# albertfgu/diffwave-sashimi

Hardware: AMD Instinct MI355X
Metric: audio samples/sec (generate.py-style reverse-diffusion sampling, T=200) (higher is better)
Workload: dtype f32-equivalent (3-term bf16 split, 6 products, fp32 accumulate); 1 GPU; wnet_h256_d36_T200; backbone=wavenet, batch_per_gpu=16, L=16000, T=200, parallelism=independent clips per GPU, no collective, sampler=hipGraph replay, on-device Philox noise

## Files before the change

### diffwave-sashimi_amd/csrc/wavenet.h

```cpp
#pragma once
#include "dws_common.h"

namespace dws {

constexpr int WN_LAYER_KC = 32;
constexpr int WN_BX3_KC = 16;

struct WnLayerArgs {
    const float* x_in;
    float* x_out;
    float* skip;
    const float* part_t;
    int part_t_bstride;
    const float* A1;
    const float* A2;
    const float* Abt;
    int abt_bstride;
    const int* step_idx;
    int abt_tstride, part_t_tstride;
    const float* Wd;
    const float* Wr;
    const float* Ws;
    const float* bias1;
    const float* bias2;
// ... 20 lines not shown
    int af_scaled;
};

int launch_fold_weight_norm(const float* v, const float* g, float* out, int O, int inner, hipStream_t s);
int launch_permute_dconv(const float* w, float* out, int C, int KC, hipStream_t s);
int launch_pack_a_frag(const float* w, float* out, int M, int K, hipStream_t s);
int launch_pack_a_frag_t(const float* w, float* out, int O, int K, hipStream_t s);
int launch_step_embed(const float* steps, const float* freq, float* emb, int B, int half, hipStream_t s);
int launch_iota_f32(float* out, int n, hipStream_t s);
int launch_linear_rows(const float* in, const float* W, const float* bias, float* out, int B, int K, int O,
                       int act, hipStream_t s, float* pre_out = nullptr);
int launch_init_conv_bwd_data(const float* g, const float* y, const float* W, float* daudio, int B, int Cin, int C, int L,
                              hipStream_t s);
int launch_init_conv(const float* audio, const float* W, const float* bias, float* x, int B, int Cin, int C, int L,
                     hipStream_t s);
int launch_wn_bias_tap(const float* Wd_all, const float* part_t, float* Abt, int NL, int B, int C, hipStream_t s);
bool wn_layer_mfma_supported(int C, int S);
int launch_wn_layer_mfma(int C, int S, const WnLayerArgs& a, hipStream_t s);
int launch_wn_layer_generic(int C, int S, const WnLayerArgs& a, hipStream_t s);
bool wn_final_mfma_supported(int S);
bool wn_layer_wino_supported(int C, int S);
int launch_wino_dconv(const float* w, float* out, int C, hipStream_t s);
int launch_wn_wino_bias(const float* Wd_all, const float* part_t, float* Abt, int NL, int B, int C, hipStream_t s);
int launch_wn_layer_wino(int C, int S, const WnLayerArgs& a, hipStream_t s);
bool wn_layer_bf16x3_supported(int C, int S);
int launch_wn_layer_bf16x3(int C, int S, const WnLayerArgs& a, hipStream_t s);
int launch_pack_a_bf16x3(const float* w, void* out, int M, int K, hipStream_t s);
int launch_wn_bias_tap_bf16(const float* Wd_all, const float* part_t, const float* bias1_all, void* Abt, int NL, int B, int C,
                            hipStream_t s);
enum { WN_SPLIT_BF16X6 = 0, WN_SPLIT_F16X3 = 1 };
inline int wn_split_terms(int split) { return split == WN_SPLIT_F16X3 ? 2 : 3; }
enum { WN_BX6_MFMA_32 = 0, WN_BX6_MFMA_G2_16 = 1, WN_BX6_MFMA_16 = 2 };
constexpr int WN_BX6_MFMA_DEFAULT = WN_BX6_MFMA_16;
bool wn_layer_bx6_supported(int C, int S);
bool wn_layer_bx6_mfma16_supported(int C, int S, int split);
int launch_wn_layer_bx6(int C, int S, const WnLayerArgs& a, int split, int mfma, hipStream_t s);
int launch_weight_scale(const float* w, size_t n, const float* bias, int nb, const float* bias_b, int nb_b, float* out, hipStream_t s);
int launch_pack_a1_bx6(const float* w, void* out, int C, int split, const float* scale, hipStream_t s);
int launch_pack_a_bx6(const float* w, void* out, int M, int K, int split, const float* scale, hipStream_t s);
int launch_gemm_bx6(const float* A, const float* B, float* C, int M, int N, int K, int split, float sa, float sb, hipStream_t s);
int launch_wn_final(int S, const WnFinalArgs& a, hipStream_t s);

}
```

### diffwave-sashimi_amd/csrc/wavenet_bx6.hip

```cpp
#include <cstdlib>
#include <type_traits>

#include "bf16_split.h"
#include "wavenet.h"
#include "wn_trace.h"

namespace dws {

#ifndef BX6_PF3
#define BX6_PF3 1
#endif
#ifndef BX6_PF2
#define BX6_PF2 2
#endif
#define BX6_PF(NT) ((NT) == 2 ? BX6_PF2 : BX6_PF3)
#ifndef BX6_T_SLOTS
#define BX6_T_SLOTS 0, 2, 3, 4, 6, 7, 9
#endif

typedef float bx6_f32x4 __attribute__((ext_vector_type(4)));

#ifdef BX6_ABL_NO_NT
#define BX6_NT 0
#else
// ... 106 lines not shown
        hipLaunchKernelGGL(pack_a_bx6_kernel<SplitBf16x3>, dim3(ceil_div(n, 256)), dim3(256), 0, s, w, (unsigned short*)out, M, K, scale);
    }
    return DWS_OK;
}

template <int C, int S, int NT>
struct Bx6Tile {
    static constexpr int WAVES = C / 32;
    static constexpr int NTH = WAVES * 64;
    static constexpr int NP = 32;
    static constexpr int KC = (C >= 256) ? 32 : 16;
    static constexpr int NCB = C / KC;
    static constexpr int NKB = C / 16;
    static constexpr int MS = S / C;
    static constexpr int RAW_FLOATS = KC * 4 * NP;
    static constexpr int BOP_BYTES = (KC / 8) * 4 * NT * NP * 16;
    static constexpr int STAGE_FLOATS = 2 * RAW_FLOATS + 2 * BOP_BYTES / 4;
    static constexpr int GATE_BYTES = (C / 8) * NT * 64 * 16;
    static constexpr int MAIN_FLOATS = STAGE_FLOATS > GATE_BYTES / 4 ? STAGE_FLOATS : GATE_BYTES / 4;
    static constexpr int TR_FLOATS = 32 * 64;
    static constexpr int LDS_FLOATS = MAIN_FLOATS + WAVES * TR_FLOATS;
    static constexpr int TITEMS = (KC / 4) * NP * 2;
    static constexpr bool HALVES = WAVES == 8 && NT == 3;
    static constexpr int SW = HALVES ? WAVES / 2 : WAVES;
    static constexpr int NPIECE = KC / (2 * SW);
    static_assert(C % 32 == 0 && S % C == 0 && C % KC == 0 && KC % 16 == 0 && KC % (2 * SW) == 0 && (SW & (SW - 1)) == 0 &&
                  (!HALVES || NCB % 2 == 0) && (TITEMS % NTH == 0) && LDS_FLOATS * 4 <= 163840, "channel counts");
};

enum { BX6_MF_32 = 0, BX6_MF_G2_16 = 1, BX6_MF_16 = 2 };
#ifndef BX6_T16_SLOTS
#define BX6_T16_SLOTS 1, 5, 7, 9, 13, 15, 19
#endif
struct Bx6Nothing {};
template <int MS>
struct Bx6G2State {
    bx_f32x4 bias[1 + MS][2];
    bx_f32x4 acc[1 + MS][2][2][2];
};
template <int NT>
__device__ __forceinline__ int bx6_voff_a1h(int lane) { return ((lane >> 5) * (4 * NT * 64) + ((lane >> 4) & 1) * 32 + (lane & 15)) * 16; }
template <typename V8, int NT>
__device__ __forceinline__ void bx6_load_a1h(V8 (&dst)[2][NT], __amdgpu_buffer_rsrc_t r, int voff, int soff) {
#pragma unroll
    for (int h = 0; h < 2; ++h)
#pragma unroll
        for (int t = 0; t < NT; ++t) dst[h][t] = __builtin_bit_cast(V8, __builtin_amdgcn_raw_buffer_load_b128(r, voff + h * 256, soff + t * 1024, 0));
}
template <typename V8, int NT>
struct Bx6G1State {
    bx_f32x4 av[2][2][4], ab[2][2];
    bx_f32x4 acc[2][4][2][2];
    V8 ar[2][2][NT];
};
template <typename P, int C, int S, bool EXTRA, int MF = BX6_MF_32>
__global__ __launch_bounds__(C * 2, (C >= 128 ? 2 : 1)) void wn_layer_bx6_kernel(WnLayerArgs a, int log2d) {
    using T = Bx6Tile<C, S, P::NT>;
    static_assert(MF == BX6_MF_32 || (P::NT == 3 && !P::SCALED && C == 256 && S == 256), "the 16x16x32 shape: bf16 split, C = S = 256");
    using v8 = typename P::v8;
    using v4 = typename P::v4;
    constexpr int NT = P::NT, NPR = P::NP, NA = 2 * P::NT;
    constexpr int KC = T::KC, MS = T::MS, WAVES = T::WAVES, NCB = T::NCB, NTH = T::NTH, NKB = T::NKB;
    __shared__ __attribute__((aligned(16))) float lds[T::LDS_FLOATS];
    float* const Xraw = lds;
    char* const Bop = reinterpret_cast<char*>(lds + 2 * T::RAW_FLOATS);
    char* const gt = reinterpret_cast<char*>(lds);

    const int tid = threadIdx.x;
    const int lane = tid & 63;
    const int wave = __builtin_amdgcn_readfirstlane(tid >> 6);
    const int l31 = lane & 31, lhi = lane >> 5;
    const int L = a.L, dil = 1 << log2d;
    float* const trw = lds + T::MAIN_FLOATS + wave * T::TR_FLOATS;

    const int nblk = (L + 2 * dil - 1) >> (log2d + 1);
    const int ntl = ((nblk << log2d) + 31) >> 5;
    const int tile = xcd_remap(blockIdx.x, gridDim.x);
    const int b = __builtin_amdgcn_readfirstlane(tile / ntl);
    const int tic = tile % ntl;
#ifdef WN_TILE_ORDER_LINEAR
    const int q0 = __builtin_amdgcn_readfirstlane(tic * 32);
#else
    const int q0 = __builtin_amdgcn_readfirstlane(log2d >= 6 ? ((tic % nblk) << log2d) + (tic / nblk) * 32 : tic * 32);
#endif
    const int q = q0 + l31;
    const int p = ((q >> log2d) << (log2d + 1)) + (q & (dil - 1));

    const float* __restrict__ xb = a.x_in + (size_t)b * C * L;
    unsigned long long* __restrict__ trc = a.trace ? a.trace + ((size_t)blockIdx.x * WAVES + wave) * 32 : nullptr;
    auto stamp = [&](int i) {
        if (trc) {
// ... 150 lines not shown
    auto transform = [&](int c1) {
        TState ts;
#pragma unroll
        for (int u = 0; u < T_UNITS; ++u) transform_unit(c1, u, ts);
    };
    auto keep_residual = [&](int c1) {
        const int ch0 = chunk_of(c1) * KC;
        if (al16 && ch0 / 32 == wave) {
            const float* xs = Xraw + (c1 & 1) * T::RAW_FLOATS;
            const int r0 = ch0 % 32;
#pragma unroll
            for (int i = 0; i < KC / 4; ++i) {
                const int rr = (lane >> 4) + 4 * i;
                const bx6_f32x4 v = *reinterpret_cast<const bx6_f32x4*>(xs + rr * 128 + 32 + 4 * (lane & 15));
                *reinterpret_cast<bx6_f32x4*>(trw + (r0 + rr) * 64 + 4 * (lane & 15)) = v;
            }
        }
    };

    bx_f32x16 acc[2][4];
    __amdgpu_buffer_rsrc_t rA1 = __builtin_amdgcn_make_buffer_rsrc((void*)a.A1, 0, 2 * C * 4 * C * 2 * NT, 0x00020000);
    const int lane16 = lane * 16;
    auto load_a1 = [&](v8 (&dst)[2][NT], int kb, int j) {
#pragma unroll
        for (int m = 0; m < 2; ++m)
#pragma unroll
            for (int t = 0; t < NT; ++t)
#ifdef BX6_ABL_A_HOT
                dst[m][t] = __builtin_bit_cast(v8, __builtin_amdgcn_raw_buffer_load_b128(rA1, lane16, ((mt1[m] * NKB * 4) * NT + t) * 1024 + 0 * (kb + j), 0));
#else
                dst[m][t] = __builtin_bit_cast(v8, __builtin_amdgcn_raw_buffer_load_b128(rA1, lane16, (((mt1[m] * NKB + kb) * 4 + j) * NT + t) * 1024, 0));
#endif
    };

    if constexpr (MF >= BX6_MF_16) {
        static_assert(T::HALVES && NCB > 1 && BX6_PF(NT) == 1 && KC == 32,
                      "a wave stages chunk 0 or chunk 1; one half-step of six fragments ahead: NAF and the chunk loop's vmcnt counts as in the 32x32x16 form");
        bx6_load_a1h<v8, NT>(gs1.ar[0], rA1, bx6_voff_a1h<NT>(lane), ((mt1[0] * NKB + 2 * chunk_of(0)) * 4 + 0) * NT * 1024);
        stage_dma(shalf);
    } else {
    if (stages(0)) stage_dma(0);
    if (NCB > 1 && stages(1)) stage_dma(1);
    }
    constexpr int PF = BX6_PF(NT);
    v8 a_ring[4][2][NT];
    if constexpr (MF < BX6_MF_16) {
#pragma unroll
    for (int s0 = 0; s0 < PF; ++s0) load_a1(a_ring[s0], chunk_of(0) * (KC / 16) + (s0 >> 2), s0 & 3);
    }
    constexpr int NAF = PF * NA;
    constexpr int P16 = NPIECE + NAF, P4 = 4 * NPIECE + NAF;
    static_assert(P4 < 64, "vmcnt is a 6-bit counter");
    if constexpr (MF >= BX6_MF_16) {
        float bi[2][4];
#pragma unroll
        for (int c = 0; c < 2; ++c) {
            const int qc = q0 + 16 * c + (lane & 15);
            const int pc = ((qc >> log2d) << (log2d + 1)) + (qc & (dil - 1));
            const float v0 = ((unsigned)(pc - dil) < (unsigned)L) ? 1.f : 0.f;
            const float v1 = ((unsigned)pc < (unsigned)L) ? 1.f : 0.f;
            const float v2 = ((unsigned)(pc + dil) < (unsigned)L) ? 1.f : 0.f;
            const float v3 = ((unsigned)(pc + 2 * dil) < (unsigned)L) ? 1.f : 0.f;
            bi[c][0] = v0 - v2; bi[c][1] = v1 + v2; bi[c][2] = v2 - v1; bi[c][3] = v1 - v3;
        }
#pragma unroll
        for (int j = 0; j < 4; ++j)
#pragma unroll
            for (int m = 0; m < 2; ++m)
#pragma unroll
                for (int h = 0; h < 2; ++h)
#pragma unroll
// ... 90 lines not shown
#pragma unroll
            for (int m = 0; m < 2; ++m) {
                acc[m][j] = P::mfma(a_ring[st & 3][m][P::ia(t)], bq[P::ib(t)], acc[m][j]);
                if (ride) {
                    const int i = 2 * t + m;
#pragma unroll
                    for (int u = 0; u < T_UNITS; ++u)
                        if (T_SLOTS[NPR == 3 ? 0 : 1][u] == i) transform_unit(cb + 1, u, ts);
                    __builtin_amdgcn_sched_barrier(0);
                }
            }
    };
    auto do_steps_from1 = [&](int cb) {
        if constexpr (SPC == 4) {
            do_step(cb, std::integral_constant<int, 1>{}, std::false_type{});
            do_step(cb, std::integral_constant<int, 2>{}, std::false_type{});
            do_step(cb, std::integral_constant<int, 3>{}, std::false_type{});
        } else {
            do_step(cb, std::integral_constant<int, 1>{}, std::false_type{});
            do_step(cb, std::integral_constant<int, 2>{}, std::false_type{});
            do_step(cb, std::integral_constant<int, 3>{}, std::false_type{});
            do_step(cb, std::integral_constant<int, 4>{}, std::false_type{});
            do_step(cb, std::integral_constant<int, 5>{}, std::false_type{});
            do_step(cb, std::integral_constant<int, 6>{}, std::false_type{});
            do_step(cb, std::integral_constant<int, 7>{}, std::false_type{});
        }
    };
    static_assert((SPC == 4 || SPC == 8) && PF >= 1 && PF <= 3, "steps per chunk, prefetch distance");
    if constexpr (MF >= BX6_MF_16) {
        const int r16 = lane & 15, oct = lane >> 4;
        const int voffa = bx6_voff_a1h<NT>(lane);
        constexpr int T16_SLOTS[T_UNITS] = {BX6_T16_SLOTS};
        v8 bq[2][NT], bq0[2][2];
        auto do_half = [&](int cb, auto HS, auto WITH_T) {
            constexpr int hs = decltype(HS)::value, j = hs >> 1, m = hs & 1;
            constexpr bool ride = decltype(WITH_T)::value;
            const char* tb = Bop + (cb & 1) * T::BOP_BYTES + oct * (4 * NT * 512) + r16 * 16;
            if (hs == 2 && cb + 1 < NCB) keep_residual(cb + 1);
            if (hs < 7) bx6_load_a1h<v8, NT>(gs1.ar[(hs + 1) & 1], rA1, voffa, ((mt1[(hs + 1) & 1] * NKB + 2 * chunk_of(cb)) * 4 + ((hs + 1) >> 1)) * NT * 1024);
            else if (cb + 1 < NCB) bx6_load_a1h<v8, NT>(gs1.ar[0], rA1, voffa, ((mt1[0] * NKB + 2 * chunk_of(cb + 1)) * 4 + 0) * NT * 1024);
            __builtin_amdgcn_sched_barrier(0);
            if (hs == 0) {
#pragma unroll
                for (int t = 0; t < NT; ++t)
#pragma unroll
                    for (int c = 0; c < 2; ++c) (t ? bq[c][t] : bq0[0][c]) = *reinterpret_cast<const v8*>(tb + (j * NT + t) * 512 + c * 256);
            }
            if (m == 1 && j < 3) {
#pragma unroll
                for (int c = 0; c < 2; ++c) bq0[(j + 1) & 1][c] = *reinterpret_cast<const v8*>(tb + ((j + 1) * NT) * 512 + c * 256);
            }
            TState ts;
#pragma unroll
            for (int t = 0; t < NPR; ++t) {
#pragma unroll
                for (int h = 0; h < 2; ++h)
#pragma unroll
                    for (int c = 0; c < 2; ++c) {
                        gs1.acc[m][j][h][c] = P::mfma16(gs1.ar[hs & 1][h][P::ia(t)], P::ib(t) ? bq[c][P::ib(t)] : bq0[j & 1][c], gs1.acc[m][j][h][c]);
                        if (ride) {
                            const int i = (2 * t + h) * 2 + c;
#pragma unroll
                            for (int u = 0; u < T_UNITS; ++u)
                                if (T16_SLOTS[u] == i) transform_unit(cb + 1, u, ts);
                            __builtin_amdgcn_sched_barrier(0);
                        }
                    }
                if (m == 1 && j < 3 && (t == 2 || t == 4)) {
                    const int term = (t == 2) ? 2 : 1;
#pragma unroll
                    for (int c = 0; c < 2; ++c) bq[c][term] = *reinterpret_cast<const v8*>(tb + ((j + 1) * NT + term) * 512 + c * 256);
                }
            }
        };
        for (int cb = 0; cb < NCB; ++cb) {
            if (cb + 2 < NCB && stages(cb + 2)) stage_dma(cb + 2);
            if (cb + 1 < NCB) do_half(cb, std::integral_constant<int, 0>{}, std::true_type{});
            else do_half(cb, std::integral_constant<int, 0>{}, std::false_type{});
            do_half(cb, std::integral_constant<int, 1>{}, std::false_type{});
            do_half(cb, std::integral_constant<int, 2>{}, std::false_type{});
            do_half(cb, std::integral_constant<int, 3>{}, std::false_type{});
            do_half(cb, std::integral_constant<int, 4>{}, std::false_type{});
            do_half(cb, std::integral_constant<int, 5>{}, std::false_type{});
            do_half(cb, std::integral_constant<int, 6>{}, std::false_type{});
            do_half(cb, std::integral_constant<int, 7>{}, std::false_type{});
            stamp(8 + 2 * cb);
            __builtin_amdgcn_s_waitcnt(0x0F70 | NAF);
            __syncthreads();
            stamp(9 + 2 * cb);
        }
    } else {
    for (int cb = 0; cb < NCB; ++cb) {
#ifndef BX6_ABL_NO_STAGE
        if (cb + 2 < NCB && stages(cb + 2)) stage_dma(cb + 2);
#endif
        if (cb + 1 < NCB) do_step(cb, std::integral_constant<int, 0>{}, std::true_type{});
        else do_step(cb, std::integral_constant<int, 0>{}, std::false_type{});
        do_steps_from1(cb);
        stamp(8 + 2 * cb);
#ifndef BX6_ABL_NO_DMA_WAIT
        __builtin_amdgcn_s_waitcnt(0x0F70 | NAF);
#endif
#ifndef BX6_ABL_NO_BARRIER
        __syncthreads();
#endif
        stamp(9 + 2 * cb);
    }
    }
    stamp(2);
    int lane_t = lane;
    if constexpr (MF >= BX6_MF_16) asm volatile("" : "+v"(lane_t));

    [[maybe_unused]] std::conditional_t<MF >= BX6_MF_G2_16, Bx6G2State<MS>, Bx6Nothing> gs2;
    if constexpr (MF >= BX6_MF_G2_16) {
#pragma unroll
        for (int m = 0; m < 1 + MS; ++m)
#pragma unroll
            for (int h = 0; h < 2; ++h) gs2.bias[m][h] = *reinterpret_cast<const bx_f32x4*>(a.bias2 + mt2[m] * 32 + 16 * h + 4 * (lane_t >> 4));
    }
    const int L4 = L * 4;
    const bool first = a.first_layer, last = a.last_layer;
    __amdgpu_buffer_rsrc_t rXo = __builtin_amdgcn_make_buffer_rsrc((void*)(a.x_out + (size_t)b * C * L), 0, C * L * 4, 0x00020000);
// ... 319 lines not shown
        }
#pragma unroll
        for (int n = 0; n < 2; ++n) {
            if (!last) {
                const int s0 = (wave * 32) * L4;
#pragma unroll
                for (int r = 0; r < 16; ++r) {
                    const int so = s0 + ((r & 3) + 8 * (r >> 2)) * L4;
                    const float x = __builtin_bit_cast(float, __builtin_amdgcn_raw_buffer_load_b32(rXall, voffn[n], so, 0));
                    const float v = (x + (P::SCALED ? acc2[0][n][r] * inv2 : acc2[0][n][r])) * rs;
                    __builtin_amdgcn_raw_buffer_store_b32(__builtin_bit_cast(unsigned, v), rXo, voffn[n], so, 0);
                }
            }
#pragma unroll
            for (int m = 0; m < MS; ++m) {
                const int s0 = ((wave * MS + m) * 32) * L4;
#pragma unroll
                for (int r = 0; r < 16; ++r) {
                    const int so = s0 + ((r & 3) + 8 * (r >> 2)) * L4;
                    const float old = first ? 0.f : __builtin_bit_cast(float, __builtin_amdgcn_raw_buffer_load_b32(rSk, voffn[n], so, 0));
                    const float v = old + (P::SCALED ? acc2[1 + m][n][r] * inv2 : acc2[1 + m][n][r]);
                    __builtin_amdgcn_raw_buffer_store_b32(__builtin_bit_cast(unsigned, v), rSk, voffn[n], so, 0);
                }
            }
        }
    }
    stamp(6);
    if (trc) {
        __builtin_amdgcn_s_waitcnt(0);
        stamp(7);
    }
}

template <typename P, int C, int S, int MF = BX6_MF_32>
static int launch_bx6_t(const WnLayerArgs& a, int log2d, hipStream_t s) {
    ProfileScope ps(P::NT == 3 ? "wn_layer_bx6" : "wn_layer_f16x3", s);
    using T = Bx6Tile<C, S, P::NT>;
    const int dil = 1 << log2d;
    const int nblk = (a.L + 2 * dil - 1) / (2 * dil);
    const int ntl = (nblk * dil + 31) / 32;
    const int ntiles = a.B * ntl;
    static const bool trace = std::getenv("DWS_BX6_TRACE") != nullptr;
    if (trace && !a.melc && !a.hsave) {
        wino_trace_launch(ntiles, T::WAVES, a, s, [&](const WnLayerArgs& at) {
            hipLaunchKernelGGL((wn_layer_bx6_kernel<P, C, S, false, MF>), dim3(ntiles), dim3(T::NTH), 0, s, at, log2d);
        }, P::NT == 3 ? "bx6" : "f16x3");
        return DWS_OK;
    }
    if (a.melc || a.hsave) hipLaunchKernelGGL((wn_layer_bx6_kernel<P, C, S, true, MF>), dim3(ntiles), dim3(T::NTH), 0, s, a, log2d);
    else hipLaunchKernelGGL((wn_layer_bx6_kernel<P, C, S, false, MF>), dim3(ntiles), dim3(T::NTH), 0, s, a, log2d);
    return DWS_OK;
}

bool wn_layer_bx6_mfma16_supported(int C, int S, int split) { return split == WN_SPLIT_BF16X6 && C == 256 && S == 256; }

bool wn_layer_bx6_supported(int C, int S) {
    return (C == 64 && S == 64) || (C == 128 && S == 128) || (C == 128 && S == 256) || (C == 256 && S == 256);
}

template <typename P>
static int launch_bx6_p(int C, int S, const WnLayerArgs& a, int log2d, hipStream_t s) {
    if (C == 64 && S == 64) return launch_bx6_t<P, 64, 64>(a, log2d, s);
    if (C == 128 && S == 128) return launch_bx6_t<P, 128, 128>(a, log2d, s);
    if (C == 128 && S == 256) return launch_bx6_t<P, 128, 256>(a, log2d, s);
    if (C == 256 && S == 256) return launch_bx6_t<P, 256, 256>(a, log2d, s);
    return set_error(DWS_ERR_UNSUPPORTED, "wn_layer_bx6: (C=%d,S=%d) not instantiated", C, S);
}

int launch_wn_layer_bx6(int C, int S, const WnLayerArgs& a, int split, int mfma, hipStream_t s) {
    int log2d = 0;
    while ((1 << log2d) < a.dilation) ++log2d;
    DWS_CHECK((1 << log2d) == a.dilation, DWS_ERR_UNSUPPORTED, "wn_layer_bx6: dilation %d is not a power of two", a.dilation);
    DWS_CHECK((int64_t)a.L + 4 * (int64_t)a.dilation < ((int64_t)1 << 28), DWS_ERR_UNSUPPORTED, "wn_layer_bx6: L too large");
    DWS_CHECK((int64_t)(C > S ? C : S) * a.L * 4 < ((int64_t)1 << 31), DWS_ERR_UNSUPPORTED,
              "wn_layer_bx6: %d channels x L=%d exceed a 2 GiB tensor per clip", C > S ? C : S, a.L);
    if (split == WN_SPLIT_F16X3) {
        DWS_CHECK(a.hsave == nullptr, DWS_ERR_UNSUPPORTED, "wn_layer_f16x3: the training forward runs with precision=f32 or bf16x6");
        DWS_CHECK(a.wscale != nullptr, DWS_ERR_INVALID, "wn_layer_f16x3: no weight scales");
        return launch_bx6_p<SplitF16x2>(C, S, a, log2d, s);
    }
    if ((mfma == WN_BX6_MFMA_G2_16 || mfma == WN_BX6_MFMA_16) && wn_layer_bx6_mfma16_supported(C, S, split)) {
        DWS_CHECK(((size_t)a.bias2 & 15) == 0, DWS_ERR_UNSUPPORTED, "wn_layer_bx6: bias2 is not 16-byte aligned");
        if (mfma == WN_BX6_MFMA_16)
            DWS_CHECK((((size_t)a.Abt | (size_t)a.bias1) & 15) == 0 && a.abt_bstride % 4 == 0 && a.abt_tstride % 4 == 0, DWS_ERR_UNSUPPORTED,
                      "wn_layer_bx6: Abt / bias1 rows are not 16-byte aligned (strides %d, %d floats)", a.abt_bstride, a.abt_tstride);
    }
    if (mfma == WN_BX6_MFMA_G2_16 && wn_layer_bx6_mfma16_supported(C, S, split)) return launch_bx6_t<SplitBf16x3, 256, 256, BX6_MF_G2_16>(a, log2d, s);
    if (mfma == WN_BX6_MFMA_16 && wn_layer_bx6_mfma16_supported(C, S, split)) return launch_bx6_t<SplitBf16x3, 256, 256, BX6_MF_16>(a, log2d, s);
    DWS_CHECK(mfma == WN_BX6_MFMA_32 || mfma == WN_BX6_MFMA_G2_16 || mfma == WN_BX6_MFMA_16, DWS_ERR_INVALID, "wn_layer_bx6: unknown MFMA shape %d", mfma);
    return launch_bx6_p<SplitBf16x3>(C, S, a, log2d, s);
}

template <typename P>
__global__ __launch_bounds__(64) void gemm_bx6_kernel(const float* __restrict__ A, const float* __restrict__ B, float* __restrict__ Cm,
                                                      int M, int N, int K, float sa, float sb) {
    using v8 = typename P::v8;
    const int lane = threadIdx.x, l31 = lane & 31, lhi = lane >> 5;
    const int mt = blockIdx.y, nt = blockIdx.x;
    bx_f32x16 acc;
#pragma unroll
    for (int r = 0; r < 16; ++r) acc[r] = 0.f;
    for (int kb = 0; kb < K / 16; ++kb) {
        v8 af[P::NT], bf[P::NT];
#pragma unroll
        for (int e = 0; e < 8; ++e) {
            const int k = kb * 16 + 8 * lhi + e;
            P::split1(A[(size_t)(mt * 32 + l31) * K + k] * sa, af, e);
            P::split1(B[(size_t)k * N + nt * 32 + l31] * sb, bf, e);
        }
#pragma unroll
        for (int t = 0; t < P::NP; ++t) acc = P::mfma(af[P::ia(t)], bf[P::ib(t)], acc);
    }
    const float inv = 1.f / (sa * sb);
#pragma unroll
    for (int r = 0; r < 16; ++r)
        Cm[(size_t)(mt * 32 + (r & 3) + 8 * (r >> 2) + 4 * lhi) * N + nt * 32 + l31] = acc[r] * inv;
}

int launch_gemm_bx6(const float* A, const float* B, float* Cm, int M, int N, int K, int split, float sa, float sb, hipStream_t s) {
    DWS_CHECK(M > 0 && N > 0 && K > 0 && M % 32 == 0 && N % 32 == 0 && K % 16 == 0, DWS_ERR_UNSUPPORTED,
              "gemm_bf16x6 / gemm_f16x3: M=%d N=%d must be multiples of 32, K=%d of 16", M, N, K);
// ... 26 lines not shown
```

### diffwave-sashimi_amd/csrc/wavenet_model.hip

```cpp
#include <cmath>

#include "conditioner.h"
#include "model.h"
#include "wavenet.h"
#include "wavenet_backward.h"

namespace dws {

struct WaveNetModel : dws_model {
    int Cin, Cout, C, S, NL, cycle, Ein, Emid, Eout, MB;
    bool cond, mfma_layer, mfma_final;
    bool bf16x3 = false;
    bool bf16x6 = false;
    bool f16x3 = false;
    DevBuf wscale;
    bool wino_opt = true;
    int bx6_mfma = WN_BX6_MFMA_DEFAULT;
    bool bx6_mfma_env_bad = false;
    static bool parse_bx6_mfma(const std::string& v, int& out) {
        if (v == "32x32x16") { out = WN_BX6_MFMA_32; return true; }
        if (v == "gemm2-16x16x32") { out = WN_BX6_MFMA_G2_16; return true; }
        if (v == "16x16x32") { out = WN_BX6_MFMA_16; return true; }
        return false;
    }
    bool wino_fits(int64_t nL) const {
        return (int64_t)std::max(C, S) * nL * 4 < ((int64_t)1 << 31) && nL + 4 * ((int64_t)1 << (cycle - 1)) < ((int64_t)1 << 28);
    }
    bool wino() const { return wino_opt && mfma_layer && !bf16x3 && !bf16x6 && !f16x3 && wn_layer_wino_supported(C, S) && (L == 0 || wino_fits(L)); }
    bool wino_rows() const { return wino() || bf16x6 || f16x3; }

    DevBuf Wi;
    std::vector<DevBuf> A1, Wrs, A2, bias2;
    DevBuf Wd_all;
    DevBuf Abt;
    DevBuf Wt_all, bt_all;
    DevBuf b1_all;
    DevBuf Wf, Af;
    DevBuf freq;
    CopyBatch stack_params, unstack_fc_t;
    bool freq_ready = false;
    DevBuf tmp_pack;
    std::vector<DevBuf> melW0, melW1, melWc;
    DevBuf melc;
    DevBuf mel_u0, mel_u1;
    int64_t melBm = 0;
    DevBuf mel_in;
    int mel_T = 0;
    CondTrainWs cws;
    DevBuf gW0f, gW1f, gWcf;
    DevBuf x0, x1, skip, gate, emb, h1, h2, part_t, scratch_out;
    std::vector<DevBuf> tx, tH;
    std::vector<DevBuf> ATd, ATg;
    std::vector<DevBuf> ATw;
    DevBuf ATf, wpart, bpart;
    bool mfma_bwd = false;
    uint64_t commit_version = 0, bwd_pack_version = ~0ull;
    DevBuf ty, ta1, ta2, dxa, dxb, dskip, dgb, dHb, dresb, dyb, dWfold, dpt, dh2, dh1, demb, dWt_all, dbt_all;
    DevBuf de_raw;
    bool trained_fwd = false;

    explicit WaveNetModel(const dws_model_desc& dd) {
        d = dd;
        Cin = d.in_channels; Cout = d.out_channels; C = d.res_channels; S = d.skip_channels;
        NL = d.num_res_layers; cycle = d.dilation_cycle;
        Ein = d.diffusion_step_embed_dim_in; Emid = d.diffusion_step_embed_dim_mid; Eout = d.diffusion_step_embed_dim_out;
        MB = d.mel_bands;
        cond = !d.unconditional;
        mfma_layer = wn_layer_mfma_supported(C, S);
        mfma_bwd = tapconv_mfma_supported(C, S, C, 1) && tapconv_mfma_supported(C, 2 * C, 0, 3) &&
                   tapconv_mfma_supported(S, S, 0, 1) && std::getenv("DWS_WAVENET_GENERIC_BWD") == nullptr;
        mfma_final = wn_final_mfma_supported(S);
        if (std::getenv("DWS_WN_DIRECT")) wino_opt = false;
        if (const char* e = std::getenv("DWS_BX6_MFMA")) bx6_mfma_env_bad = !parse_bx6_mfma(e, bx6_mfma);
        auto wn = [&](const std::string& p, std::vector<int64_t> vshape) {
            std::vector<int64_t> g(vshape.size(), 1);
            g[0] = vshape[0];
            add_param(p + ".bias", {vshape[0]});
            add_param(p + ".weight_g", g);
            add_param(p + ".weight_v", vshape);
        };
        wn("init_conv.0.conv", {C, Cin, 1});
        add_param("residual_layer.fc_t1.weight", {Emid, Ein});
        add_param("residual_layer.fc_t1.bias", {Emid});
        add_param("residual_layer.fc_t2.weight", {Eout, Emid});
        add_param("residual_layer.fc_t2.bias", {Eout});
        for (int n = 0; n < NL; ++n) {
            const std::string p = "residual_layer.residual_blocks." + std::to_string(n);
            add_param(p + ".fc_t.weight", {C, Eout});
            add_param(p + ".fc_t.bias", {C});
            wn(p + ".dilated_conv_layer.conv", {2 * C, C, 3});
            if (cond) {
                for (int i = 0; i < 2; ++i) {
                    const std::string u = p + ".upsample_conv2d." + std::to_string(i);
                    const int s = d.mel_upsample[i];
                    add_param(u + ".bias", {1});
                    add_param(u + ".weight_g", {1, 1, 1, 1});
                    add_param(u + ".weight_v", {1, 1, 3, 2 * s});
                }
                wn(p + ".mel_conv.conv", {2 * C, MB, 1});
            }
            wn(p + ".res_conv", {C, C, 1});
            wn(p + ".skip_conv", {S, C, 1});
        }
        wn("final_conv.0.conv", {S, S, 1});
        add_param("final_conv.2.conv.weight", {Cout, S, 1});
        add_param("final_conv.2.conv.bias", {Cout});
// ... 4 lines not shown

    int set_option(const std::string& key, const std::string& value) override {
        if (key == "precision") {
            if (value == "f32") { bf16x3 = bf16x6 = f16x3 = false; dirty = true; trained_fwd = false; return DWS_OK; }
            if (value == "bf16x3") {
                DWS_CHECK(wn_layer_bf16x3_supported(C, S), DWS_ERR_UNSUPPORTED,
                          "precision=bf16x3 is not built for (res_channels=%d, skip_channels=%d)", C, S);
                bf16x3 = true; bf16x6 = f16x3 = false; dirty = true; trained_fwd = false;
                return DWS_OK;
            }
            if (value == "bf16x6") {
                DWS_CHECK(mfma_layer && wn_layer_bx6_supported(C, S), DWS_ERR_UNSUPPORTED,
                          "precision=bf16x6 is not built for (res_channels=%d, skip_channels=%d)", C, S);
                bf16x6 = true; bf16x3 = f16x3 = false; dirty = true; trained_fwd = false;
                return DWS_OK;
            }
            if (value == "f16x3") {
                DWS_CHECK(mfma_layer && wn_layer_bx6_supported(C, S), DWS_ERR_UNSUPPORTED,
                          "precision=f16x3 is not built for (res_channels=%d, skip_channels=%d)", C, S);
                f16x3 = true; bf16x3 = bf16x6 = false; dirty = true; trained_fwd = false;
                return DWS_OK;
            }
        }
        if (key == "conv_algo") {
            if (value == "winograd") { wino_opt = true; dirty = true; trained_fwd = false; return DWS_OK; }
            if (value == "direct") { wino_opt = false; dirty = true; trained_fwd = false; return DWS_OK; }
        }
        if (key == "bx6_mfma") {
            int v = 0;
            DWS_CHECK(parse_bx6_mfma(value, v), DWS_ERR_INVALID, "bx6_mfma: 32x32x16 | gemm2-16x16x32 | 16x16x32, not '%s'", value.c_str());
            bx6_mfma = v; bx6_mfma_env_bad = false; dirty = true; trained_fwd = false;
            return DWS_OK;
        }
        return dws_model::set_option(key, value);
    }

    float* Wd(int n) const { return Wd_all.f() + (size_t)n * 2 * C * C * 3; }

    int fold(const std::string& p, float* out, int O, int inner, hipStream_t s) {
        return launch_fold_weight_norm(P(p + ".weight_v"), P(p + ".weight_g"), out, O, inner, s);
    }

    int commit(hipStream_t s) override {
        DWS_CHECK(!bx6_mfma_env_bad, DWS_ERR_INVALID, "DWS_BX6_MFMA: 32x32x16 | gemm2-16x16x32 | 16x16x32, not '%s'", std::getenv("DWS_BX6_MFMA") ? std::getenv("DWS_BX6_MFMA") : "");
        DWS_TRY(Wi.ensure((size_t)C * Cin * 4));
        DWS_TRY(fold("init_conv.0.conv", Wi.f(), C, Cin, s));
        DWS_TRY(Wt_all.ensure((size_t)NL * C * Eout * 4));
        DWS_TRY(bt_all.ensure((size_t)NL * C * 4));
        DWS_TRY(b1_all.ensure((size_t)NL * 2 * C * 4));
        DWS_TRY(Wd_all.ensure((size_t)NL * 2 * C * C * 3 * 4));
        if (mfma_layer) DWS_TRY(tmp_pack.ensure((size_t)2 * C * 4 * C * 4));
        stack_params.begin();
        for (int n = 0; n < NL; ++n) {
            const std::string p = "residual_layer.residual_blocks." + std::to_string(n);
            stack_params.add(P(p + ".fc_t.weight"), Wt_all.f() + (size_t)n * C * Eout, (size_t)C * Eout);
            stack_params.add(P(p + ".fc_t.bias"), bt_all.f() + (size_t)n * C, (size_t)C);
            stack_params.add(P(p + ".dilated_conv_layer.conv.bias"), b1_all.f() + (size_t)n * 2 * C, (size_t)2 * C);
            DWS_TRY(fold(p + ".dilated_conv_layer.conv", Wd(n), 2 * C, C * 3, s));
            DWS_TRY(Wrs[n].ensure((size_t)(C + S) * C * 4));
            DWS_TRY(fold(p + ".res_conv", Wrs[n].f(), C, C, s));
            DWS_TRY(fold(p + ".skip_conv", Wrs[n].f() + (size_t)C * C, S, C, s));
            DWS_TRY(bias2[n].ensure((size_t)(C + S) * 4));
            stack_params.add(P(p + ".res_conv.bias"), bias2[n].f(), (size_t)C);
            stack_params.add(P(p + ".skip_conv.bias"), bias2[n].f() + C, (size_t)S);
            if (mfma_layer && (bf16x6 || f16x3)) {
                const int split = f16x3 ? WN_SPLIT_F16X3 : WN_SPLIT_BF16X6;
                const size_t tb = 2 * (size_t)wn_split_terms(split);
                float* sc = nullptr;
                if (f16x3) {
                    DWS_TRY(wscale.ensure((size_t)NL * 2 * 4));
                    sc = wscale.f() + 2 * n;
                    DWS_TRY(launch_weight_scale(Wd(n), (size_t)2 * C * C * 3, P(p + ".dilated_conv_layer.conv.bias"), 2 * C, nullptr, 0, sc, s));
                    DWS_TRY(launch_weight_scale(Wrs[n].f(), (size_t)(C + S) * C, P(p + ".res_conv.bias"), C, P(p + ".skip_conv.bias"), S,
                                                sc + 1, s));
                }
                DWS_TRY(A1[n].ensure((size_t)2 * C * 4 * C * tb));
                DWS_TRY(A2[n].ensure((size_t)(C + S) * C * tb));
// ... 323 lines not shown
                                           tab_rep > 1 ? NL * C : 0, step_idx, tab_rep * NL * C, s);
            return launch_wn_mask_tail(x, lengths_ptr(), (int)B, C, (int)L, reach, part_t.f() + (size_t)n * C, NL * C, nullptr, 0, s);
        };
        const bool rag = ragged() && !train;
        if (rag) DWS_TRY(seal(xfirst, 0));
        for (int n = 0; n < NL; ++n) {
            const std::string p = "residual_layer.residual_blocks." + std::to_string(n);
            WnLayerArgs a{};
            a.x_in = train ? tx[n].f() : ((n & 1) ? x1.f() : x0.f());
            a.x_out = train ? tx[n + 1].f() : ((n & 1) ? x0.f() : x1.f());
            a.hsave = train ? tH[n].f() : nullptr;
            a.skip = skip.f();
            a.A1 = A1[n].f(); a.A2 = A2[n].f();
            if (tab) {
                const int pb = tab_rep > 1 ? NL * C : 0, ab = tab_rep > 1 ? arow : 0;
                a.part_t = tab_pt.f() + (size_t)n * C; a.part_t_bstride = pb; a.part_t_tstride = tab_rep * NL * C;
                a.Abt = mfma_layer ? tab_abt.f() + (size_t)n * tab_T * tab_rep * arow : nullptr; a.abt_bstride = ab;
                a.abt_tstride = tab_rep * arow;
                a.step_idx = step_idx;
            } else {
                a.part_t = part_t.f() + (size_t)n * C; a.part_t_bstride = NL * C;
                a.Abt = mfma_layer ? Abt.f() + (size_t)n * B * arow : nullptr; a.abt_bstride = arow;
            }
            a.Wd = Wd(n); a.Wr = Wrs[n].f(); a.Ws = Wrs[n].f() + (size_t)C * C;
            a.bias1 = P(p + ".dilated_conv_layer.conv.bias");
            a.bias2 = bias2[n].f();
            a.melc = melBm ? melc.f() + (size_t)n * melBm * 2 * C * L : nullptr;
            a.mel_bstride = (melBm > 1) ? 1 : 0;
            a.gate_ws = gate.f();
            a.B = (int)B; a.L = (int)L;
            a.dilation = 1 << (n % cycle);
            a.first_layer = (n == 0); a.last_layer = (n == NL - 1);
            if (mfma_layer && bf16x3) DWS_TRY(launch_wn_layer_bf16x3(C, S, a, s));
            else if (bf16x6) DWS_TRY(launch_wn_layer_bx6(C, S, a, WN_SPLIT_BF16X6, bx6_mfma, s));
            else if (f16x3) { a.wscale = wscale.f() + 2 * n; DWS_TRY(launch_wn_layer_bx6(C, S, a, WN_SPLIT_F16X3, WN_BX6_MFMA_32, s)); }
            else if (wino()) DWS_TRY(launch_wn_layer_wino(C, S, a, s));
            else if (mfma_layer) DWS_TRY(launch_wn_layer_mfma(C, S, a, s));
            else DWS_TRY(launch_wn_layer_generic(C, S, a, s));
            if (rag && n + 1 < NL) DWS_TRY(seal(a.x_out, n + 1));
        }
        DWS_TRY(final_stage(out, train ? ty.f() : nullptr, s));
        if (rag) DWS_TRY(launch_wn_mask_tail(out, lengths_ptr(), (int)B, Cout, (int)L, -1, nullptr, 0, nullptr, 0, s));
        DWS_HIP(hipGetLastError());
        return DWS_OK;
    }

    int wn_bwd(const std::string& p, const float* dWf, int O, int inner, hipStream_t s) {
        return launch_weight_norm_bwd(dWf, P(p + ".weight_v"), P(p + ".weight_g"), G(p + ".weight_v"), G(p + ".weight_g"), O,
                                      inner, s);
    }

    int backward(const float* dout, float* daudio, bool pg, hipStream_t s) override {
        DWS_CHECK(trained_fwd, DWS_ERR_STATE, "backward without a preceding forward_train");
        DWS_CHECK(pg || daudio, DWS_ERR_INVALID, "backward: a data-only pass needs a destination for the input gradient");
        const int nB = (int)B, nL = (int)L;
        const size_t act = (size_t)B * C * L * 4, nact = (size_t)B * C * L;
        DWS_TRY(dxa.ensure(act)); DWS_TRY(dxb.ensure(act)); DWS_TRY(dgb.ensure(act)); DWS_TRY(dresb.ensure(act));
        DWS_TRY(gate.ensure(act));
        DWS_TRY(dHb.ensure(2 * act));
        DWS_TRY(dskip.ensure((size_t)B * S * L * 4)); DWS_TRY(dyb.ensure((size_t)B * S * L * 4));
        if (pg) {
            DWS_TRY(dWfold.ensure((size_t)std::max(2 * C * C * 3, std::max((C + S) * C, S * S)) * 4));
            DWS_TRY(dpt.ensure((size_t)B * NL * C * 4));
            DWS_TRY(dh2.ensure((size_t)B * Eout * 4)); DWS_TRY(dh1.ensure((size_t)B * Emid * 4));
            DWS_TRY(dWt_all.ensure((size_t)NL * C * Eout * 4)); DWS_TRY(dbt_all.ensure((size_t)NL * C * 4));
        }
        const float scale = (float)std::sqrt(1.0 / NL);

// ... 185 lines not shown
```

Before: 33990 audio samples/s.

## Prefetch GEMM1 A fragments through a quarter-step ring with configurable lead

Adds a quarter-step A-operand ring for the 16x16x32 bx6 GEMM1 path, made the default. A fragments are now requested in quarter-step sets up to BX6_A_LEAD quarters ahead, crossing into the next channel block, instead of one half-step set at a time. The aim is finer-grained global-load latency hiding behind the MFMA stream. The cost is a different vmcnt wait depth and more in-flight registers, which could raise register pressure or change how the scheduler interleaves work. Both the env var and the option API can select it.

```diff
diff --git a/diffwave-sashimi_amd/csrc/wavenet.h b/diffwave-sashimi_amd/csrc/wavenet.h
--- a/diffwave-sashimi_amd/csrc/wavenet.h
+++ b/diffwave-sashimi_amd/csrc/wavenet.h
@@ -76,9 +76,11 @@
 inline int wn_split_terms(int split) { return split == WN_SPLIT_F16X3 ? 2 : 3; }
 enum { WN_BX6_MFMA_32 = 0, WN_BX6_MFMA_G2_16 = 1, WN_BX6_MFMA_16 = 2 };
 constexpr int WN_BX6_MFMA_DEFAULT = WN_BX6_MFMA_16;
+enum { WN_BX6_A_RING_HALF = 0, WN_BX6_A_RING_QUARTER = 1 };
+constexpr int WN_BX6_A_RING_DEFAULT = WN_BX6_A_RING_QUARTER;
 bool wn_layer_bx6_supported(int C, int S);
 bool wn_layer_bx6_mfma16_supported(int C, int S, int split);
-int launch_wn_layer_bx6(int C, int S, const WnLayerArgs& a, int split, int mfma, hipStream_t s);
+int launch_wn_layer_bx6(int C, int S, const WnLayerArgs& a, int split, int mfma, int a_ring, hipStream_t s);
 int launch_weight_scale(const float* w, size_t n, const float* bias, int nb, const float* bias_b, int nb_b, float* out, hipStream_t s);
 int launch_pack_a1_bx6(const float* w, void* out, int C, int split, const float* scale, hipStream_t s);
 int launch_pack_a_bx6(const float* w, void* out, int M, int K, int split, const float* scale, hipStream_t s);
diff --git a/diffwave-sashimi_amd/csrc/wavenet_bx6.hip b/diffwave-sashimi_amd/csrc/wavenet_bx6.hip
--- a/diffwave-sashimi_amd/csrc/wavenet_bx6.hip
+++ b/diffwave-sashimi_amd/csrc/wavenet_bx6.hip
@@ -162,6 +162,10 @@
 #ifndef BX6_T16_SLOTS
 #define BX6_T16_SLOTS 1, 5, 7, 9, 13, 15, 19
 #endif
+enum { BX6_AR_HALF = 0, BX6_AR_QUARTER = 1 };
+#ifndef BX6_A_LEAD
+#define BX6_A_LEAD 3
+#endif
 struct Bx6Nothing {};
 template <int MS>
 struct Bx6G2State {
@@ -178,15 +182,22 @@
         for (int t = 0; t < NT; ++t) dst[h][t] = __builtin_bit_cast(V8, __builtin_amdgcn_raw_buffer_load_b128(r, voff + h * 256, soff + t * 1024, 0));
 }
 template <typename V8, int NT>
+__device__ __forceinline__ void bx6_load_a1q(V8 (&dst)[NT], __amdgpu_buffer_rsrc_t r, int voff, int soff) {
+#pragma unroll
+    for (int t = 0; t < NT; ++t) dst[t] = __builtin_bit_cast(V8, __builtin_amdgcn_raw_buffer_load_b128(r, voff, soff + t * 1024, 0));
+}
+template <typename V8, int NT>
 struct Bx6G1State {
     bx_f32x4 av[2][2][4], ab[2][2];
     bx_f32x4 acc[2][4][2][2];
     V8 ar[2][2][NT];
 };
-template <typename P, int C, int S, bool EXTRA, int MF = BX6_MF_32>
+template <typename P, int C, int S, bool EXTRA, int MF = BX6_MF_32, int AR = BX6_AR_HALF>
 __global__ __launch_bounds__(C * 2, (C >= 128 ? 2 : 1)) void wn_layer_bx6_kernel(WnLayerArgs a, int log2d) {
     using T = Bx6Tile<C, S, P::NT>;
     static_assert(MF == BX6_MF_32 || (P::NT == 3 && !P::SCALED && C == 256 && S == 256), "the 16x16x32 shape: bf16 split, C = S = 256");
+    static_assert(AR == BX6_AR_HALF || MF >= BX6_MF_16, "the quarter-step A ring belongs to the 16x16x32 GEMM1");
+    static_assert(BX6_A_LEAD >= 1 && BX6_A_LEAD <= 3, "quarter-step ring of four sets: a lead of four would request into the set in use");
     using v8 = typename P::v8;
     using v4 = typename P::v4;
     constexpr int NT = P::NT, NPR = P::NP, NA = 2 * P::NT;
@@ -403,11 +414,21 @@
                 dst[m][t] = __builtin_bit_cast(v8, __builtin_amdgcn_raw_buffer_load_b128(rA1, lane16, (((mt1[m] * NKB + kb) * 4 + j) * NT + t) * 1024, 0));
 #endif
     };
+    [[maybe_unused]] auto req_a1q = [&](int cbi, int qq) __attribute__((always_inline)) {
+        if constexpr (MF >= BX6_MF_16)
+            bx6_load_a1q<v8, NT>(gs1.ar[(qq >> 1) & 1][qq & 1], rA1, bx6_voff_a1h<NT>(lane) + (qq & 1) * 256,
+                                 ((mt1[(qq >> 1) & 1] * NKB + 2 * chunk_of(cbi)) * 4 + (qq >> 2)) * NT * 1024);
+    };
 
     if constexpr (MF >= BX6_MF_16) {
         static_assert(T::HALVES && NCB > 1 && BX6_PF(NT) == 1 && KC == 32,
                       "a wave stages chunk 0 or chunk 1; one half-step of six fragments ahead: NAF and the chunk loop's vmcnt counts as in the 32x32x16 form");
+        if constexpr (AR == BX6_AR_QUARTER) {
+#pragma unroll
+            for (int qq = 0; qq < BX6_A_LEAD; ++qq) req_a1q(0, qq);
+        } else {
         bx6_load_a1h<v8, NT>(gs1.ar[0], rA1, bx6_voff_a1h<NT>(lane), ((mt1[0] * NKB + 2 * chunk_of(0)) * 4 + 0) * NT * 1024);
+        }
         stage_dma(shalf);
     } else {
     if (stages(0)) stage_dma(0);
@@ -564,6 +585,79 @@
         const int voffa = bx6_voff_a1h<NT>(lane);
         constexpr int T16_SLOTS[T_UNITS] = {BX6_T16_SLOTS};
         v8 bq[2][NT], bq0[2][2];
+        if constexpr (AR == BX6_AR_QUARTER) {
+        constexpr int LEAD = BX6_A_LEAD, QPC = 16;
+        auto do_quarter = [&](int cb, auto QS, auto WITH_T, TState& ts) __attribute__((always_inline)) {
+            constexpr int qs = decltype(QS)::value, j = qs >> 2, m = (qs >> 1) & 1, h = qs & 1;
+            constexpr bool ride = decltype(WITH_T)::value;
+            constexpr bool lastq = m == 1 && h == 1;
+            const char* tb = Bop + (cb & 1) * T::BOP_BYTES + oct * (4 * NT * 512) + r16 * 16;
+            if (qs == 4 && cb + 1 < NCB) keep_residual(cb + 1);
+            __builtin_amdgcn_sched_barrier(0);
+            if (qs + LEAD < QPC) req_a1q(cb, qs + LEAD);
+            else if (cb + 1 < NCB) req_a1q(cb + 1, qs + LEAD - QPC);
+            __builtin_amdgcn_sched_barrier(0);
+            if (qs == 0) {
+#pragma unroll
+                for (int t = 0; t < NT; ++t)
+#pragma unroll
+                    for (int c = 0; c < 2; ++c) (t ? bq[c][t] : bq0[0][c]) = *reinterpret_cast<const v8*>(tb + (j * NT + t) * 512 + c * 256);
+            }
+            if (lastq && j < 3) {
+#pragma unroll
+                for (int c = 0; c < 2; ++c) bq0[(j + 1) & 1][c] = *reinterpret_cast<const v8*>(tb + ((j + 1) * NT) * 512 + c * 256);
+            }
+#pragma unroll
+            for (int t = 0; t < NPR; ++t) {
+#pragma unroll
+                for (int c = 0; c < 2; ++c) {
+                    gs1.acc[m][j][h][c] = P::mfma16(gs1.ar[m][h][P::ia(t)], P::ib(t) ? bq[c][P::ib(t)] : bq0[j & 1][c], gs1.acc[m][j][h][c]);
+                    if (ride) {
+                        const int i = 12 * qs + 2 * t + c;
+#pragma unroll
+                        for (int u = 0; u < T_UNITS; ++u)
+                            if (T16_SLOTS[u] == i) transform_unit(cb + 1, u, ts);
+                        __builtin_amdgcn_sched_barrier(0);
+                    }
+                }
+                if (lastq && j < 3 && (t == 2 || t == 4)) {
+                    const int term = (t == 2) ? 2 : 1;
+#pragma unroll
+                    for (int c = 0; c < 2; ++c) bq[c][term] = *reinterpret_cast<const v8*>(tb + ((j + 1) * NT + term) * 512 + c * 256);
+                }
+            }
+        };
+        for (int cb = 0; cb < NCB; ++cb) {
+            if (cb + 2 < NCB && stages(cb + 2)) stage_dma(cb + 2);
+            TState ts;
+            if (cb + 1 < NCB) {
+                do_quarter(cb, std::integral_constant<int, 0>{}, std::true_type{}, ts);
+                do_quarter(cb, std::integral_constant<int, 1>{}, std::true_type{}, ts);
+            } else {
+                do_quarter(cb, std::integral_constant<int, 0>{}, std::false_type{}, ts);
+                do_quarter(cb, std::integral_constant<int, 1>{}, std::false_type{}, ts);
+            }
+            do_quarter(cb, std::integral_constant<int, 2>{}, std::false_type{}, ts);
+            do_quarter(cb, std::integral_constant<int, 3>{}, std::false_type{}, ts);
+            do_quarter(cb, std::integral_constant<int, 4>{}, std::false_type{}, ts);
+            do_quarter(cb, std::integral_constant<int, 5>{}, std::false_type{}, ts);
+            do_quarter(cb, std::integral_constant<int, 6>{}, std::false_type{}, ts);
+            do_quarter(cb, std::integral_constant<int, 7>{}, std::false_type{}, ts);
+            do_quarter(cb, std::integral_constant<int, 8>{}, std::false_type{}, ts);
+            do_quarter(cb, std::integral_constant<int, 9>{}, std::false_type{}, ts);
+            do_quarter(cb, std::integral_constant<int, 10>{}, std::false_type{}, ts);
+            do_quarter(cb, std::integral_constant<int, 11>{}, std::false_type{}, ts);
+            do_quarter(cb, std::integral_constant<int, 12>{}, std::false_type{}, ts);
+            do_quarter(cb, std::integral_constant<int, 13>{}, std::false_type{}, ts);
+            do_quarter(cb, std::integral_constant<int, 14>{}, std::false_type{}, ts);
+            do_quarter(cb, std::integral_constant<int, 15>{}, std::false_type{}, ts);
+            stamp(8 + 2 * cb);
+            static_assert(3 * LEAD < 16, "vmcnt immediate: low four bits only");
+            __builtin_amdgcn_s_waitcnt(0x0F70 | (NT * LEAD));
+            __syncthreads();
+            stamp(9 + 2 * cb);
+        }
+        } else {
         auto do_half = [&](int cb, auto HS, auto WITH_T) {
             constexpr int hs = decltype(HS)::value, j = hs >> 1, m = hs & 1;
             constexpr bool ride = decltype(WITH_T)::value;
@@ -620,6 +714,7 @@
             __builtin_amdgcn_s_waitcnt(0x0F70 | NAF);
             __syncthreads();
             stamp(9 + 2 * cb);
+        }
         }
     } else {
     for (int cb = 0; cb < NCB; ++cb) {
@@ -1005,7 +1100,7 @@
     }
 }
 
-template <typename P, int C, int S, int MF = BX6_MF_32>
+template <typename P, int C, int S, int MF = BX6_MF_32, int AR = BX6_AR_HALF>
 static int launch_bx6_t(const WnLayerArgs& a, int log2d, hipStream_t s) {
     ProfileScope ps(P::NT == 3 ? "wn_layer_bx6" : "wn_layer_f16x3", s);
     using T = Bx6Tile<C, S, P::NT>;
@@ -1016,12 +1111,12 @@
     static const bool trace = std::getenv("DWS_BX6_TRACE") != nullptr;
     if (trace && !a.melc && !a.hsave) {
         wino_trace_launch(ntiles, T::WAVES, a, s, [&](const WnLayerArgs& at) {
-            hipLaunchKernelGGL((wn_layer_bx6_kernel<P, C, S, false, MF>), dim3(ntiles), dim3(T::NTH), 0, s, at, log2d);
+            hipLaunchKernelGGL((wn_layer_bx6_kernel<P, C, S, false, MF, AR>), dim3(ntiles), dim3(T::NTH), 0, s, at, log2d);
         }, P::NT == 3 ? "bx6" : "f16x3");
         return DWS_OK;
     }
-    if (a.melc || a.hsave) hipLaunchKernelGGL((wn_layer_bx6_kernel<P, C, S, true, MF>), dim3(ntiles), dim3(T::NTH), 0, s, a, log2d);
-    else hipLaunchKernelGGL((wn_layer_bx6_kernel<P, C, S, false, MF>), dim3(ntiles), dim3(T::NTH), 0, s, a, log2d);
+    if (a.melc || a.hsave) hipLaunchKernelGGL((wn_layer_bx6_kernel<P, C, S, true, MF, AR>), dim3(ntiles), dim3(T::NTH), 0, s, a, log2d);
+    else hipLaunchKernelGGL((wn_layer_bx6_kernel<P, C, S, false, MF, AR>), dim3(ntiles), dim3(T::NTH), 0, s, a, log2d);
     return DWS_OK;
 }
 
@@ -1040,7 +1135,7 @@
     return set_error(DWS_ERR_UNSUPPORTED, "wn_layer_bx6: (C=%d,S=%d) not instantiated", C, S);
 }
 
-int launch_wn_layer_bx6(int C, int S, const WnLayerArgs& a, int split, int mfma, hipStream_t s) {
+int launch_wn_layer_bx6(int C, int S, const WnLayerArgs& a, int split, int mfma, int a_ring, hipStream_t s) {
     int log2d = 0;
     while ((1 << log2d) < a.dilation) ++log2d;
     DWS_CHECK((1 << log2d) == a.dilation, DWS_ERR_UNSUPPORTED, "wn_layer_bx6: dilation %d is not a power of two", a.dilation);
@@ -1059,7 +1154,11 @@
                       "wn_layer_bx6: Abt / bias1 rows are not 16-byte aligned (strides %d, %d floats)", a.abt_bstride, a.abt_tstride);
     }
     if (mfma == WN_BX6_MFMA_G2_16 && wn_layer_bx6_mfma16_supported(C, S, split)) return launch_bx6_t<SplitBf16x3, 256, 256, BX6_MF_G2_16>(a, log2d, s);
-    if (mfma == WN_BX6_MFMA_16 && wn_layer_bx6_mfma16_supported(C, S, split)) return launch_bx6_t<SplitBf16x3, 256, 256, BX6_MF_16>(a, log2d, s);
+    DWS_CHECK(a_ring == WN_BX6_A_RING_HALF || a_ring == WN_BX6_A_RING_QUARTER, DWS_ERR_INVALID, "wn_layer_bx6: unknown A ring %d", a_ring);
+    if (mfma == WN_BX6_MFMA_16 && wn_layer_bx6_mfma16_supported(C, S, split)) {
+        if (a_ring == WN_BX6_A_RING_QUARTER) return launch_bx6_t<SplitBf16x3, 256, 256, BX6_MF_16, BX6_AR_QUARTER>(a, log2d, s);
+        return launch_bx6_t<SplitBf16x3, 256, 256, BX6_MF_16>(a, log2d, s);
+    }
     DWS_CHECK(mfma == WN_BX6_MFMA_32 || mfma == WN_BX6_MFMA_G2_16 || mfma == WN_BX6_MFMA_16, DWS_ERR_INVALID, "wn_layer_bx6: unknown MFMA shape %d", mfma);
     return launch_bx6_p<SplitBf16x3>(C, S, a, log2d, s);
 }
diff --git a/diffwave-sashimi_amd/csrc/wavenet_model.hip b/diffwave-sashimi_amd/csrc/wavenet_model.hip
--- a/diffwave-sashimi_amd/csrc/wavenet_model.hip
+++ b/diffwave-sashimi_amd/csrc/wavenet_model.hip
@@ -21,6 +21,13 @@
         if (v == "32x32x16") { out = WN_BX6_MFMA_32; return true; }
         if (v == "gemm2-16x16x32") { out = WN_BX6_MFMA_G2_16; return true; }
         if (v == "16x16x32") { out = WN_BX6_MFMA_16; return true; }
+        return false;
+    }
+    int bx6_a_ring = WN_BX6_A_RING_DEFAULT;
+    bool bx6_a_ring_env_bad = false;
+    static bool parse_bx6_a_ring(const std::string& v, int& out) {
+        if (v == "half-step") { out = WN_BX6_A_RING_HALF; return true; }
+        if (v == "quarter-step") { out = WN_BX6_A_RING_QUARTER; return true; }
         return false;
     }
     bool wino_fits(int64_t nL) const {
@@ -72,6 +79,7 @@
         mfma_final = wn_final_mfma_supported(S);
         if (std::getenv("DWS_WN_DIRECT")) wino_opt = false;
         if (const char* e = std::getenv("DWS_BX6_MFMA")) bx6_mfma_env_bad = !parse_bx6_mfma(e, bx6_mfma);
+        if (const char* e = std::getenv("DWS_BX6_A_RING")) bx6_a_ring_env_bad = !parse_bx6_a_ring(e, bx6_a_ring);
         auto wn = [&](const std::string& p, std::vector<int64_t> vshape) {
             std::vector<int64_t> g(vshape.size(), 1);
             g[0] = vshape[0];
@@ -142,6 +150,12 @@
             bx6_mfma = v; bx6_mfma_env_bad = false; dirty = true; trained_fwd = false;
             return DWS_OK;
         }
+        if (key == "bx6_a_ring") {
+            int v = 0;
+            DWS_CHECK(parse_bx6_a_ring(value, v), DWS_ERR_INVALID, "bx6_a_ring: half-step | quarter-step, not '%s'", value.c_str());
+            bx6_a_ring = v; bx6_a_ring_env_bad = false; dirty = true; trained_fwd = false;
+            return DWS_OK;
+        }
         return dws_model::set_option(key, value);
     }
 
@@ -153,6 +167,7 @@
 
     int commit(hipStream_t s) override {
         DWS_CHECK(!bx6_mfma_env_bad, DWS_ERR_INVALID, "DWS_BX6_MFMA: 32x32x16 | gemm2-16x16x32 | 16x16x32, not '%s'", std::getenv("DWS_BX6_MFMA") ? std::getenv("DWS_BX6_MFMA") : "");
+        DWS_CHECK(!bx6_a_ring_env_bad, DWS_ERR_INVALID, "DWS_BX6_A_RING: half-step | quarter-step, not '%s'", std::getenv("DWS_BX6_A_RING") ? std::getenv("DWS_BX6_A_RING") : "");
         DWS_TRY(Wi.ensure((size_t)C * Cin * 4));
         DWS_TRY(fold("init_conv.0.conv", Wi.f(), C, Cin, s));
         DWS_TRY(Wt_all.ensure((size_t)NL * C * Eout * 4));
@@ -542,8 +557,8 @@
             a.dilation = 1 << (n % cycle);
             a.first_layer = (n == 0); a.last_layer = (n == NL - 1);
             if (mfma_layer && bf16x3) DWS_TRY(launch_wn_layer_bf16x3(C, S, a, s));
-            else if (bf16x6) DWS_TRY(launch_wn_layer_bx6(C, S, a, WN_SPLIT_BF16X6, bx6_mfma, s));
-            else if (f16x3) { a.wscale = wscale.f() + 2 * n; DWS_TRY(launch_wn_layer_bx6(C, S, a, WN_SPLIT_F16X3, WN_BX6_MFMA_32, s)); }
+            else if (bf16x6) DWS_TRY(launch_wn_layer_bx6(C, S, a, WN_SPLIT_BF16X6, bx6_mfma, bx6_a_ring, s));
+            else if (f16x3) { a.wscale = wscale.f() + 2 * n; DWS_TRY(launch_wn_layer_bx6(C, S, a, WN_SPLIT_F16X3, WN_BX6_MFMA_32, WN_BX6_A_RING_HALF, s)); }
             else if (wino()) DWS_TRY(launch_wn_layer_wino(C, S, a, s));
             else if (mfma_layer) DWS_TRY(launch_wn_layer_mfma(C, S, a, s));
             else DWS_TRY(launch_wn_layer_generic(C, S, a, s));
```

Result: faster. 34410 audio samples/s (median of 6 runs) (+1.2%).
